# yuriyvnv/speech_transcript_embeddings

Hardware: AMD Instinct MI355X
Metric: audio–text pairs/sec (whole node), 10s@16kHz + 64-tok, 1/2/4/8 MI355X (higher is better)
Workload: dtype bf16; 1 GPU; c2: global batch 64 = 1 GPU x 1 micro-batch(es) of 64 pairs, each pair 10s@16kHz audio + 64-tok clean + 64-tok corrupt; w2v-bert-2.0 Conformer 24L + XLM-R-base 12L, 3+3 unfrozen; GPU fbank -> fwd -> InfoNCE -> bwd -> allreduce -> clip+AdamW; global_batch=64, local_batch=64, micro_batch=64, accumulation_steps=1, seq_len_audio_frames=499, seq_len_text=64, parallelism=dp1

## Files before the change

### speech_transcript_embeddings_amd/csrc/layernorm.hip

```cpp
#include "common.h"
#include "../../include/ste.h"

namespace {

constexpr int NT = 256;

template <int MAXC>
STE_DEV void load_row(const void* base, bool is_bf16, int64_t ld, int row, int cols, int lane, float (&v)[MAXC * 4]) {
#pragma unroll
  for (int c = 0; c < MAXC; ++c) {
    int col = (lane + c * 64) * 4;
    f32x4 x = {0.f, 0.f, 0.f, 0.f};
    if (col < cols) {
      if (is_bf16) x = load_bf16x4((const bf16*)base + (int64_t)row * ld + col);
      else x = *reinterpret_cast<const f32x4*>((const float*)base + (int64_t)row * ld + col);
    }
#pragma unroll
    for (int e = 0; e < 4; ++e) v[c * 4 + e] = x[e];
  }
}

template <int MAXC>
struct LnParams {
  f32x4 g[MAXC], b[MAXC];
  STE_DEV void load(const float* gamma, const float* beta, int cols, int lane) {
#pragma unroll
    for (int c = 0; c < MAXC; ++c) {
      const int col = (lane + c * 64) * 4;
      g[c] = col < cols ? *reinterpret_cast<const f32x4*>(gamma + col) : f32x4{0.f, 0.f, 0.f, 0.f};
      b[c] = (beta && col < cols) ? *reinterpret_cast<const f32x4*>(beta + col) : f32x4{0.f, 0.f, 0.f, 0.f};
    }
  }
};

template <int MAXC>
STE_DEV void ln_fwd_row(const ste_ln_fwd_args& a, const LnParams<MAXC>& pr, int row, int lane, float (&v)[MAXC * 4]) {
  const float inv_n = 1.0f / (float)a.cols;
  const uint32_t thresh = (uint32_t)(a.drop_p * 4294967296.0);
  const float inv_keep = a.drop_p > 0.f ? 1.0f / (1.0f - a.drop_p) : 1.0f;
  float s = 0.f;
#pragma unroll
  for (int i = 0; i < MAXC * 4; ++i) s += v[i];
  const float mean = wave_sum(s) * inv_n;
  float q = 0.f;
#pragma unroll
  for (int c = 0; c < MAXC; ++c) {
    int col = (lane + c * 64) * 4;
    if (col < a.cols) {
#pragma unroll
      for (int e = 0; e < 4; ++e) { float d = v[c * 4 + e] - mean; q += d * d; }
    }
  }
  const float rstd = rsqrtf(wave_sum(q) * inv_n + a.eps);
  if (lane == 0) { a.mean[row] = mean; a.rstd[row] = rstd; }
  const float rs = a.row_scale ? a.row_scale[row] : 1.0f;
#pragma unroll
  for (int c = 0; c < MAXC; ++c) {
    int col = (lane + c * 64) * 4;
    if (col >= a.cols) continue;
    const f32x4 g = pr.g[c], b = pr.b[c];
    f32x4 y;
#pragma unroll
    for (int e = 0; e < 4; ++e) {
      float t = ((v[c * 4 + e] - mean) * rstd * g[e] + b[e]) * rs;
      if (a.act == STE_ACT_SWISH) t = swish_f(t);
      if (a.drop_p > 0.f) t *= drop_scale(a.seed, (uint64_t)row * a.cols + col + e, thresh, inv_keep);
      y[e] = t;
      v[c * 4 + e] = t;
    }
    if (a.y) *reinterpret_cast<f32x4*>(a.y + (int64_t)row * a.ldy + col) = y;
    if (a.ylo) store_bf16x4_split((bf16*)a.yb + (int64_t)row * a.ldyb + col, (bf16*)a.ylo + (int64_t)row * a.ldylo + col, y);
    else if (a.yb) store_bf16x4((bf16*)a.yb + (int64_t)row * a.ldyb + col, y);
    if (a.q8) {
      float am = fmaxf(fmaxf(fabsf(y[0]), fabsf(y[1])), fmaxf(fabsf(y[2]), fabsf(y[3])));
      am = fmaxf(am, dpp_f<0xB1>(am));
      am = fmaxf(am, dpp_f<0x4E>(am));
      am = fmaxf(am, dpp_f<0x141>(am));
      const int ex = mx8_exp(am);
      const float inv = ldexpf(1.0f, -ex);
      uint32_t w = 0;
      w = __builtin_amdgcn_cvt_pk_fp8_f32(fminf(fmaxf(y[0] * inv, -448.f), 448.f),
                                          fminf(fmaxf(y[1] * inv, -448.f), 448.f), w, false);
      w = __builtin_amdgcn_cvt_pk_fp8_f32(fminf(fmaxf(y[2] * inv, -448.f), 448.f),
                                          fminf(fmaxf(y[3] * inv, -448.f), 448.f), w, true);
      *reinterpret_cast<uint32_t*>((uint8_t*)a.q8 + (int64_t)row * a.ldq8 + col) = w;
      if ((lane & 7) == 0) ((uint8_t*)a.q8s)[(int64_t)row * (a.cols >> 5) + (col >> 5)] = (uint8_t)(ex + 127);
    }
  }
}

template <int MAXC>
__global__ __launch_bounds__(NT) void ln_fwd_kernel(ste_ln_fwd_args a) {
  const int lane = threadIdx.x & 63;
  const int wave = blockIdx.x * (NT / 64) + (threadIdx.x >> 6);
  const int nwaves = gridDim.x * (NT / 64);
  LnParams<MAXC> pa;
  pa.load(a.gamma, a.beta, a.cols, lane);
  for (int row = wave; row < a.rows; row += nwaves) {
    float v[MAXC * 4];
    load_row<MAXC>(a.x, a.x_bf16, a.ldx, row, a.cols, lane, v);
    ln_fwd_row<MAXC>(a, pa, row, lane, v);
  }
}

template <int MAXC, bool LEAN = false>
__global__ __launch_bounds__(NT) void ln_fwd_pair_kernel(ste_ln_fwd_args a, ste_ln_fwd_args b) {
  const int lane = threadIdx.x & 63;
  const int wave = blockIdx.x * (NT / 64) + (threadIdx.x >> 6);
  const int nwaves = gridDim.x * (NT / 64);
  if constexpr (LEAN) {
    for (int row = wave; row < a.rows; row += nwaves) {
      float v[MAXC * 4];
      load_row<MAXC>(a.x, a.x_bf16, a.ldx, row, a.cols, lane, v);
      const float *ga = a.gamma, *ba = a.beta, *gb = b.gamma, *bb = b.beta;
      asm volatile("" : "+s"(ga), "+s"(ba), "+s"(gb), "+s"(bb));
      {
        LnParams<MAXC> pa;
        pa.load(ga, ba, a.cols, lane);
        ln_fwd_row<MAXC>(a, pa, row, lane, v);
      }
      LnParams<MAXC> pb;
      pb.load(gb, bb, b.cols, lane);
      ln_fwd_row<MAXC>(b, pb, row, lane, v);
    }
  } else {
    LnParams<MAXC> pa;
    pa.load(a.gamma, a.beta, a.cols, lane);
    LnParams<MAXC> pb;
    pb.load(b.gamma, b.beta, b.cols, lane);
    float v[MAXC * 4], nx[MAXC * 4];
    if (wave < a.rows) load_row<MAXC>(a.x, a.x_bf16, a.ldx, wave, a.cols, lane, v);
    for (int row = wave; row < a.rows; row += nwaves) {
      if (row + nwaves < a.rows) load_row<MAXC>(a.x, a.x_bf16, a.ldx, row + nwaves, a.cols, lane, nx);
      ln_fwd_row<MAXC>(a, pa, row, lane, v);
      ln_fwd_row<MAXC>(b, pb, row, lane, v);
#pragma unroll
      for (int i = 0; i < MAXC * 4; ++i) v[i] = nx[i];
    }
  }
}
bool ln_fwd_pair_lean() {
  static int v = -1;
  if (v < 0) {
    const char* e = STE_AB_ENV("STE_LN_FWD_PAIR");
    v = (e && e[0] == 'p') ? 0 : 1;
  }
  return v == 1;
}

template <int MAXC>
struct LnAcc {
  float dg[MAXC * 4], db[MAXC * 4], dsm[MAXC * 4];
  STE_DEV void zero() {
#pragma unroll
    for (int i = 0; i < MAXC * 4; ++i) { dg[i] = 0.f; db[i] = 0.f; dsm[i] = 0.f; }
  }
};

template <int MAXC, bool PRE, bool DRPRE = PRE>
STE_DEV void ln_bwd_row(const ste_ln_bwd_args& a, int row, int lane, float (&x)[MAXC * 4], float (&g)[MAXC * 4],
                        const float* dr, const LnParams<MAXC>* pr, LnAcc<MAXC>& acc) {
  const float inv_n = 1.0f / (float)a.cols;
  const uint32_t thresh = (uint32_t)(a.drop_p * 4294967296.0);
  const float inv_keep = a.drop_p > 0.f ? 1.0f / (1.0f - a.drop_p) : 1.0f;
  const uint32_t in_thresh = (uint32_t)(a.in_drop_p * 4294967296.0);
  const float in_inv_keep = a.in_drop_p > 0.f ? 1.0f / (1.0f - a.in_drop_p) : 1.0f;
  const float mean = a.mean[row], rstd = a.rstd[row];
  const float rs = a.row_scale ? a.row_scale[row] : 1.0f;
  float s1 = 0.f, s2 = 0.f;
#pragma unroll
  for (int c = 0; c < MAXC; ++c) {
    int col = (lane + c * 64) * 4;
    if (col >= a.cols) continue;
    f32x4 gm, bt = {0.f, 0.f, 0.f, 0.f};
    if constexpr (PRE) {
      gm = pr->g[c];
      bt = pr->b[c];
    } else {
      gm = *reinterpret_cast<const f32x4*>(a.gamma + col);
      if (a.act == STE_ACT_SWISH) bt = *reinterpret_cast<const f32x4*>(a.beta + col);
    }
#pragma unroll
    for (int e = 0; e < 4; ++e) {
      const int i = c * 4 + e;
      const float xh = (x[i] - mean) * rstd;
      float gi = g[i];
      if (a.in_drop_p > 0.f) gi *= drop_scale(a.in_seed, (uint64_t)row * a.cols + col + e, in_thresh, in_inv_keep);
      if (a.act == STE_ACT_SWISH) gi *= swish_d((xh * gm[e] + bt[e]) * rs);
      gi *= rs;
      acc.dg[i] += gi * xh;
      acc.db[i] += gi;
      const float gg = gi * gm[e];
      g[i] = gg;
      x[i] = xh;
      s1 += gg;
      s2 += gg * xh;
    }
  }
  s1 = wave_sum(s1) * inv_n;
  s2 = wave_sum(s2) * inv_n;
  const float ors = a.out_row_scale ? a.out_row_scale[row] : 1.0f;
#pragma unroll
  for (int c = 0; c < MAXC; ++c) {
    int col = (lane + c * 64) * 4;
    if (col >= a.cols) continue;
    f32x4 d;
#pragma unroll
    for (int e = 0; e < 4; ++e) {
      const int i = c * 4 + e;
      d[e] = rstd * (g[i] - s1 - x[i] * s2);
    }
    if (a.dres) {
      if (DRPRE) {
#pragma unroll
        for (int e = 0; e < 4; ++e) d[e] += dr[c * 4 + e];
      } else {
        d += *reinterpret_cast<const f32x4*>(a.dres + (int64_t)row * a.lddres + col);
      }
    }
    if (a.dx) *reinterpret_cast<f32x4*>(a.dx + (int64_t)row * a.lddx + col) = d;
    if (a.dxb || a.dsum) {
      f32x4 o = d * (a.out_scale * ors);
      if (a.drop_p > 0.f) {
#pragma unroll
        for (int e = 0; e < 4; ++e) o[e] *= drop_scale(a.seed, (uint64_t)row * a.cols + col + e, thresh, inv_keep);
      }
      if (a.dxb) store_bf16x4((bf16*)a.dxb + (int64_t)row * a.lddxb + col, o);
#pragma unroll
      for (int e = 0; e < 4; ++e) acc.dsm[c * 4 + e] += o[e];
    }
#pragma unroll
    for (int e = 0; e < 4; ++e) g[c * 4 + e] = d[e];
  }
}

template <int MAXC>
STE_DEV void ln_flush(const ste_ln_bwd_args& a, const LnAcc<MAXC>& acc, float (*red)[MAXC * 4 * 64], int lane,
                      int wid) {
  float* const outs[3] = {a.dgamma, a.dbeta, a.dsum};
#pragma unroll
  for (int k = 0; k < 3; ++k) {
    if (!outs[k]) continue;
    const float* src = k == 0 ? acc.dg : (k == 1 ? acc.db : acc.dsm);
    __syncthreads();
#pragma unroll
    for (int i = 0; i < MAXC * 4; ++i) red[wid][(i >> 2) * 256 + lane * 4 + (i & 3)] = src[i];
    __syncthreads();
    float* part = a.ws ? a.ws + ((int64_t)k * gridDim.x + blockIdx.x) * a.cols : nullptr;
    for (int j = threadIdx.x; j < MAXC * 256; j += NT) {
      const int c = j >> 8, rem = j & 255;
      const int col = (c * 64 + (rem >> 2)) * 4 + (rem & 3);
      if (col >= a.cols) continue;
      float sum = 0.f;
#pragma unroll
      for (int w = 0; w < NT / 64; ++w) sum += red[w][j];
      if (part) part[col] = sum;
      else atomicAdd(outs[k] + col, sum);
    }
  }
}

constexpr int CS_CW = 16, CS_SL = 1024 / CS_CW;
__global__ __launch_bounds__(1024) void ln_colsum_kernel(const float* __restrict__ ws, int nblk, int cols,
                                                         float* dgamma, float* dbeta, float* dsum) {
  float* const out = blockIdx.y == 0 ? dgamma : (blockIdx.y == 1 ? dbeta : dsum);
  if (!out) return;
  __shared__ float red[CS_SL][CS_CW];
  const int c = threadIdx.x % CS_CW, sl = threadIdx.x / CS_CW;
  const int col = blockIdx.x * CS_CW + c;
  float acc = 0.f;
  if (col < cols) {
    const float* p = ws + (int64_t)blockIdx.y * nblk * cols + col;
    int b = sl;
    for (; b + 7 * CS_SL < nblk; b += 8 * CS_SL) {
      float v[8];
#pragma unroll
      for (int u = 0; u < 8; ++u) v[u] = p[(int64_t)(b + CS_SL * u) * cols];
#pragma unroll
      for (int u = 0; u < 8; ++u) acc += v[u];
    }
    for (; b < nblk; b += CS_SL) acc += p[(int64_t)b * cols];
  }
  red[sl][c] = acc;
  __syncthreads();
  if (sl == 0 && col < cols) {
    float t = red[0][c];
    for (int k = 1; k < CS_SL; ++k) t += red[k][c];
    out[col] += t;
  }
}

template <int MAXC, bool REDUCE>
__global__ __launch_bounds__(NT, REDUCE ? 3 : 1) void ln_bwd_kernel(ste_ln_bwd_args a) {
  __shared__ float red[REDUCE ? NT / 64 : 1][REDUCE ? MAXC * 4 * 64 : 1];
  const int lane = threadIdx.x & 63, wid = threadIdx.x >> 6;
  const int wave = blockIdx.x * (NT / 64) + wid;
  const int nwaves = gridDim.x * (NT / 64);
  LnAcc<MAXC> acc;
  acc.zero();
  LnParams<MAXC> pa;
  if constexpr (!REDUCE) pa.load(a.gamma, a.act == STE_ACT_SWISH ? a.beta : nullptr, a.cols, lane);
  for (int row = wave; row < a.rows; row += nwaves) {
    float x[MAXC * 4], g[MAXC * 4], dr[MAXC * 4];
    load_row<MAXC>(a.x, a.x_bf16, a.ldx, row, a.cols, lane, x);
    load_row<MAXC>(a.dy, a.dy_bf16, a.lddy, row, a.cols, lane, g);
    if (a.dres) load_row<MAXC>(a.dres, false, a.lddres, row, a.cols, lane, dr);
    if constexpr (REDUCE) ln_bwd_row<MAXC, false, true>(a, row, lane, x, g, dr, nullptr, acc);
    else ln_bwd_row<MAXC, true>(a, row, lane, x, g, dr, &pa, acc);
  }
  if constexpr (REDUCE) ln_flush<MAXC>(a, acc, red, lane, wid);
}

template <int MAXC, bool REDUCE>
__global__ __launch_bounds__(NT, REDUCE ? 1 : 4) void ln_bwd_pair_kernel(ste_ln_bwd_args a, ste_ln_bwd_args b) {
  __shared__ float red[REDUCE ? NT / 64 : 1][REDUCE ? MAXC * 4 * 64 : 1];
  const int lane = threadIdx.x & 63, wid = threadIdx.x >> 6;
  const int wave = blockIdx.x * (NT / 64) + wid;
  const int nwaves = gridDim.x * (NT / 64);
  LnAcc<MAXC> acc_a, acc_b;
  acc_a.zero();
  acc_b.zero();
  for (int row = wave; row < a.rows; row += nwaves) {
    float x[MAXC * 4], g[MAXC * 4], dr[MAXC * 4];
    load_row<MAXC>(b.x, b.x_bf16, b.ldx, row, b.cols, lane, x);
    load_row<MAXC>(b.dy, b.dy_bf16, b.lddy, row, b.cols, lane, g);
    if (!REDUCE && b.dres) load_row<MAXC>(b.dres, false, b.lddres, row, b.cols, lane, dr);
    ln_bwd_row<MAXC, false, !REDUCE>(b, row, lane, x, g, dr, nullptr, acc_b);
    load_row<MAXC>(a.x, a.x_bf16, a.ldx, row, a.cols, lane, x);
    ln_bwd_row<MAXC, false>(a, row, lane, x, g, nullptr, nullptr, acc_a);
  }
  if constexpr (REDUCE) {
    ln_flush<MAXC>(b, acc_b, red, lane, wid);
    ln_flush<MAXC>(a, acc_a, red, lane, wid);
  }
}

inline int grid_for(int rows, int cap = 1024) {
  int g = (rows + 3) / 4;
  return g < cap ? g : cap;
}
constexpr int LN_REDUCE_BLOCKS = 768, LN_PAIR_REDUCE_BLOCKS = 512;
inline int grid_bwd(const ste_ln_bwd_args& a, bool reduce) {
  return grid_for(a.rows, reduce ? LN_REDUCE_BLOCKS : 1024);
}
inline bool ws_ok(const ste_ln_bwd_args& a, int nblk) {
  return !a.ws || a.ws_floats >= 3 * (int64_t)nblk * a.cols;
}
inline void colsum(const ste_ln_bwd_args& a, int nblk, hipStream_t s) {
  if (!a.ws || !(a.dgamma || a.dbeta || a.dsum)) return;
  hipLaunchKernelGGL(ln_colsum_kernel, dim3((unsigned)((a.cols + CS_CW - 1) / CS_CW), 3), dim3(1024), 0, s, (const float*)a.ws,
                     nblk, a.cols, a.dgamma, a.dbeta, a.dsum);
}

}

extern "C" int ste_layernorm_fwd(const ste_ln_fwd_args* a, void* stream) {
  if (!a || a->rows <= 0 || a->cols <= 0 || (a->cols & 3) || a->cols > 2048 || !a->mean || !a->rstd)
    return STE_ERR_ARG;
  if (a->ylo && !a->yb) return STE_ERR_ARG;
  if (a->q8 && (!a->q8s || (a->cols & 127) || a->ldq8 < a->cols || (a->ldq8 & 3) || (((uintptr_t)a->q8) & 3)))
    return STE_ERR_SHAPE;
  hipStream_t s = (hipStream_t)stream;
  dim3 grid(grid_for(a->rows));
  if (a->cols <= 256) hipLaunchKernelGGL(ln_fwd_kernel<1>, grid, dim3(NT), 0, s, *a);
  else if (a->cols <= 1024) hipLaunchKernelGGL(ln_fwd_kernel<4>, grid, dim3(NT), 0, s, *a);
  else hipLaunchKernelGGL(ln_fwd_kernel<8>, grid, dim3(NT), 0, s, *a);
  STE_CHECK_LAUNCH();
  return 0;
}

extern "C" int ste_layernorm_fwd_pair(const ste_ln_fwd_args* a, const ste_ln_fwd_args* b, void* stream) {
  if (!a || !b || a->rows <= 0 || a->cols <= 0 || (a->cols & 3) || a->cols > 1024 || b->rows != a->rows ||
      b->cols != a->cols || !a->mean || !a->rstd || !b->mean || !b->rstd)
    return STE_ERR_ARG;
  for (const ste_ln_fwd_args* t : {a, b}) {
    if (t->ylo && !t->yb) return STE_ERR_ARG;
    if (t->q8 && (!t->q8s || (t->cols & 127) || t->ldq8 < t->cols || (t->ldq8 & 3) || (((uintptr_t)t->q8) & 3)))
      return STE_ERR_SHAPE;
  }
  hipStream_t s = (hipStream_t)stream;
  dim3 grid(grid_for(a->rows));
  if (a->cols <= 256) hipLaunchKernelGGL(ln_fwd_pair_kernel<1>, grid, dim3(NT), 0, s, *a, *b);
  else if (ln_fwd_pair_lean()) hipLaunchKernelGGL((ln_fwd_pair_kernel<4, true>), grid, dim3(NT), 0, s, *a, *b);
  else hipLaunchKernelGGL(ln_fwd_pair_kernel<4>, grid, dim3(NT), 0, s, *a, *b);
  STE_CHECK_LAUNCH();
  return 0;
}

extern "C" int ste_layernorm_bwd_pair(const ste_ln_bwd_args* a, const ste_ln_bwd_args* b, void* stream) {
  if (!a || !b || a->rows <= 0 || a->cols <= 0 || (a->cols & 3) || a->cols > 1024 || b->rows != a->rows ||
      b->cols != a->cols)
    return STE_ERR_ARG;
  if ((a->act == STE_ACT_SWISH && !a->beta) || (b->act == STE_ACT_SWISH && !b->beta)) return STE_ERR_ARG;
  hipStream_t s = (hipStream_t)stream;
  const bool reduce = a->dgamma || a->dbeta || a->dsum || b->dgamma || b->dbeta || b->dsum;
  const bool use_ws = (a->ws || !(a->dgamma || a->dbeta || a->dsum)) && (b->ws || !(b->dgamma || b->dbeta || b->dsum));
  const int nblk = grid_for(a->rows, reduce ? LN_PAIR_REDUCE_BLOCKS : 1024);
  if (reduce && use_ws && (!ws_ok(*a, nblk) || !ws_ok(*b, nblk))) return STE_ERR_ARG;
  ste_ln_bwd_args aa = *a, bb = *b;
  if (!use_ws) aa.ws = bb.ws = nullptr;
  const dim3 grid(nblk);
  if (a->cols <= 256) {
    if (reduce) hipLaunchKernelGGL((ln_bwd_pair_kernel<1, true>), grid, dim3(NT), 0, s, aa, bb);
    else hipLaunchKernelGGL((ln_bwd_pair_kernel<1, false>), grid, dim3(NT), 0, s, aa, bb);
  } else {
    if (reduce) hipLaunchKernelGGL((ln_bwd_pair_kernel<4, true>), grid, dim3(NT), 0, s, aa, bb);
    else hipLaunchKernelGGL((ln_bwd_pair_kernel<4, false>), grid, dim3(NT), 0, s, aa, bb);
  }
  STE_CHECK_LAUNCH();
  if (reduce && use_ws) {
    colsum(bb, nblk, s);
    colsum(aa, nblk, s);
    STE_CHECK_LAUNCH();
  }
  return 0;
}

extern "C" int ste_layernorm_bwd(const ste_ln_bwd_args* a, void* stream) {
  if (!a || a->rows <= 0 || a->cols <= 0 || (a->cols & 3) || a->cols > 1024) return STE_ERR_ARG;
  if (a->act == STE_ACT_SWISH && !a->beta) return STE_ERR_ARG;
  hipStream_t s = (hipStream_t)stream;
  const bool reduce = a->dgamma || a->dbeta || a->dsum;
  const int nblk = grid_bwd(*a, reduce);
  if (reduce && !ws_ok(*a, nblk)) return STE_ERR_ARG;
  const dim3 grid(nblk);
  if (a->cols <= 256) {
    if (reduce) hipLaunchKernelGGL((ln_bwd_kernel<1, true>), grid, dim3(NT), 0, s, *a);
    else hipLaunchKernelGGL((ln_bwd_kernel<1, false>), grid, dim3(NT), 0, s, *a);
  } else {
    if (reduce) hipLaunchKernelGGL((ln_bwd_kernel<4, true>), grid, dim3(NT), 0, s, *a);
    else hipLaunchKernelGGL((ln_bwd_kernel<4, false>), grid, dim3(NT), 0, s, *a);
  }
  STE_CHECK_LAUNCH();
  if (reduce) {
    colsum(*a, nblk, s);
    STE_CHECK_LAUNCH();
  }
  return 0;
}

extern "C" int64_t ste_layernorm_bwd_ws_floats(int rows, int cols) {
  return rows <= 0 || cols <= 0 ? 0 : 3 * (int64_t)grid_for(rows, LN_REDUCE_BLOCKS) * cols;
}
```

Before: 494.7 pairs/s.

## Add LDS ring-buffered LayerNorm forward pair kernel using global_load_lds prefetch

Adds a new paired LayerNorm forward kernel that prefetches the next row of fp32 input (plus row scales) straight into a per-wave LDS slot with global_load_lds. It keeps gamma/beta for both norms in shared memory instead of registers, and uses explicit vmcnt waits so the next row's loads overlap the current row's compute and stores. The aim is to hide load latency and lower register pressure (launch bounds allow 4 blocks). It is used by default for fp32 inputs with 512–1024 columns and no fp8 output, and the old path stays selectable through an env var. It relies on hand-written asm waitcnt counting, which is fragile if the store count estimate is wrong.

```diff
diff --git a/profiles/ln_dma_probe.py b/profiles/ln_dma_probe.py
--- /dev/null
+++ b/profiles/ln_dma_probe.py
@@ -0,0 +1,88 @@
+import argparse
+import json
+import os
+import statistics
+import sys
+from pathlib import Path
+
+import torch
+
+sys.path.insert(0, str(Path(__file__).resolve().parents[1]))
+from speech_transcript_embeddings_amd import _lib, ops
+
+M, D = 31936, 1024
+BF16 = torch.bfloat16
+
+
+def timed(fn, iters):
+    fn()
+    torch.cuda.synchronize()
+    e0, e1 = torch.cuda.Event(enable_timing=True), torch.cuda.Event(enable_timing=True)
+    e0.record()
+    for _ in range(iters):
+        fn()
+    e1.record()
+    torch.cuda.synchronize()
+    return round(e0.elapsed_time(e1) * 1e3 / iters, 2)
+
+
+def cases():
+    dev = "cuda"
+    torch.manual_seed(0)
+    x = torch.randn(M, D, device=dev)
+    x5s = torch.randn(M, 2 * D, device=dev)
+    g, b = 1 + 0.1 * torch.randn(D, device=dev), 0.1 * torch.randn(D, device=dev)
+    g2, b2 = 1 + 0.1 * torch.randn(D, device=dev), 0.1 * torch.randn(D, device=dev)
+    rs = (torch.rand(M, device=dev) > 0.1).float()
+    y = torch.empty(M, D, device=dev)
+    yb2 = torch.empty(M, D, device=dev, dtype=BF16)
+    ys = torch.empty(M, 2 * D, device=dev, dtype=BF16)
+    mean, rstd = torch.empty(M, device=dev), torch.empty(M, device=dev)
+    m2, r2 = torch.empty(M, device=dev), torch.empty(M, device=dev)
+    c = {}
+    c["fwd_pair ring: y+yb+ylo | yb"] = (1, lambda: ops.layernorm_fwd_pair(
+        dict(x=x, gamma=g, beta=b, eps=1e-5, y=y, yb=ys[:, :D], ylo=ys[:, D:], mean=mean, rstd=rstd),
+        dict(gamma=g2, beta=b2, eps=1e-5, yb=yb2, mean=m2, rstd=r2)), (y, ys, yb2, mean, rstd, m2, r2))
+    c["fwd_pair ring: wide x, y+yb+ylo | yb row_scale"] = (1, lambda: ops.layernorm_fwd_pair(
+        dict(x=x5s[:, :D], gamma=g, beta=b, eps=1e-5, y=y, yb=ys[:, :D], ylo=ys[:, D:], mean=mean, rstd=rstd),
+        dict(gamma=g2, beta=b2, eps=1e-5, yb=yb2, mean=m2, rstd=r2, row_scale=rs)), (y, ys, yb2, mean, rstd, m2, r2))
+    return c
+
+
+def main():
+    ap = argparse.ArgumentParser()
+    ap.add_argument("--iters", type=int, default=20)
+    ap.add_argument("--alt", type=int, default=7)
+    ap.add_argument("--out", default=None)
+    a = ap.parse_args()
+    assert _lib.AB_BUILD, "run with STE_LIB=.../libste_ab.so (python -m speech_transcript_embeddings_amd._build --ab)"
+    lines = []
+    for name, (bit, fn, outs) in cases().items():
+        old, new = [], []
+        for _ in range(a.alt):
+            os.environ["STE_LN_DMA"] = "0"
+            old.append(timed(fn, a.iters))
+            os.environ["STE_LN_DMA"] = str(bit)
+            new.append(timed(fn, a.iters))
+        os.environ["STE_LN_DMA"] = "0"
+        fn()
+        ref = [t.clone() for t in outs]
+        for t in outs:
+            t.fill_(3.0)
+        os.environ["STE_LN_DMA"] = str(bit)
+        fn()
+        torch.cuda.synchronize()
+        same = all(torch.equal(r, t) for r, t in zip(ref, outs))
+        res = dict(case=name, rows=M, cols=D, parent_us=old, ring_us=new, parent_median=statistics.median(old),
+                   ring_median=statistics.median(new), parent_spread=round(max(old) - min(old), 2),
+                   ring_spread=round(max(new) - min(new), 2), bit_identical=same)
+        res["speedup"] = round(res["parent_median"] / res["ring_median"], 3)
+        lines.append(json.dumps(res))
+        print(lines[-1], flush=True)
+    if a.out:
+        Path(a.out).parent.mkdir(parents=True, exist_ok=True)
+        Path(a.out).write_text("\n".join(lines) + "\n")
+
+
+if __name__ == "__main__":
+    main()
diff --git a/speech_transcript_embeddings_amd/csrc/layernorm.hip b/speech_transcript_embeddings_amd/csrc/layernorm.hip
--- a/speech_transcript_embeddings_amd/csrc/layernorm.hip
+++ b/speech_transcript_embeddings_amd/csrc/layernorm.hip
@@ -1,9 +1,15 @@
+#include <cstdlib>
 #include "common.h"
 #include "../../include/ste.h"
 
 namespace {
 
 constexpr int NT = 256;
+
+inline int grid_for(int rows, int cap = 1024) {
+  int g = (rows + 3) / 4;
+  return g < cap ? g : cap;
+}
 
 template <int MAXC>
 STE_DEV void load_row(const void* base, bool is_bf16, int64_t ld, int row, int cols, int lane, float (&v)[MAXC * 4]) {
@@ -31,10 +37,13 @@
       b[c] = (beta && col < cols) ? *reinterpret_cast<const f32x4*>(beta + col) : f32x4{0.f, 0.f, 0.f, 0.f};
     }
   }
+  STE_DEV void get(int c, f32x4& gc, f32x4& bc) const { gc = g[c]; bc = b[c]; }
 };
 
-template <int MAXC>
-STE_DEV void ln_fwd_row(const ste_ln_fwd_args& a, const LnParams<MAXC>& pr, int row, int lane, float (&v)[MAXC * 4]) {
+STE_DEV float fwd_rs(const ste_ln_fwd_args& a, int row) { return a.row_scale ? a.row_scale[row] : 1.0f; }
+template <int MAXC, class Params>
+STE_DEV void ln_fwd_row(const ste_ln_fwd_args& a, const Params& pr, int row, int lane, float (&v)[MAXC * 4],
+                        float rs) {
   const float inv_n = 1.0f / (float)a.cols;
   const uint32_t thresh = (uint32_t)(a.drop_p * 4294967296.0);
   const float inv_keep = a.drop_p > 0.f ? 1.0f / (1.0f - a.drop_p) : 1.0f;
@@ -53,12 +62,12 @@
   }
   const float rstd = rsqrtf(wave_sum(q) * inv_n + a.eps);
   if (lane == 0) { a.mean[row] = mean; a.rstd[row] = rstd; }
-  const float rs = a.row_scale ? a.row_scale[row] : 1.0f;
 #pragma unroll
   for (int c = 0; c < MAXC; ++c) {
     int col = (lane + c * 64) * 4;
     if (col >= a.cols) continue;
-    const f32x4 g = pr.g[c], b = pr.b[c];
+    f32x4 g, b;
+    pr.get(c, g, b);
     f32x4 y;
 #pragma unroll
     for (int e = 0; e < 4; ++e) {
@@ -99,7 +108,7 @@
   for (int row = wave; row < a.rows; row += nwaves) {
     float v[MAXC * 4];
     load_row<MAXC>(a.x, a.x_bf16, a.ldx, row, a.cols, lane, v);
-    ln_fwd_row<MAXC>(a, pa, row, lane, v);
+    ln_fwd_row<MAXC>(a, pa, row, lane, v, fwd_rs(a, row));
   }
 }
 
@@ -117,11 +126,11 @@
       {
         LnParams<MAXC> pa;
         pa.load(ga, ba, a.cols, lane);
-        ln_fwd_row<MAXC>(a, pa, row, lane, v);
+        ln_fwd_row<MAXC>(a, pa, row, lane, v, fwd_rs(a, row));
       }
       LnParams<MAXC> pb;
       pb.load(gb, bb, b.cols, lane);
-      ln_fwd_row<MAXC>(b, pb, row, lane, v);
+      ln_fwd_row<MAXC>(b, pb, row, lane, v, fwd_rs(b, row));
     }
   } else {
     LnParams<MAXC> pa;
@@ -132,8 +141,8 @@
     if (wave < a.rows) load_row<MAXC>(a.x, a.x_bf16, a.ldx, wave, a.cols, lane, v);
     for (int row = wave; row < a.rows; row += nwaves) {
       if (row + nwaves < a.rows) load_row<MAXC>(a.x, a.x_bf16, a.ldx, row + nwaves, a.cols, lane, nx);
-      ln_fwd_row<MAXC>(a, pa, row, lane, v);
-      ln_fwd_row<MAXC>(b, pb, row, lane, v);
+      ln_fwd_row<MAXC>(a, pa, row, lane, v, fwd_rs(a, row));
+      ln_fwd_row<MAXC>(b, pb, row, lane, v, fwd_rs(b, row));
 #pragma unroll
       for (int i = 0; i < MAXC * 4; ++i) v[i] = nx[i];
     }
@@ -148,6 +157,118 @@
   return v == 1;
 }
 
+typedef __attribute__((address_space(3))) const char lds_cchar;
+STE_DEV uint32_t lds_off(const void* p) { return (uint32_t)(uintptr_t)(lds_cchar*)p; }
+
+template <int N>
+STE_DEV void lds_read_chunks(uint32_t off, f32x4 (&r)[N]) {
+  static_assert(N >= 2 && N <= 4, "2..4 chunks");
+  if constexpr (N == 2)
+    asm volatile("ds_read_b128 %0, %2\n\tds_read_b128 %1, %2 offset:1024\n\ts_waitcnt lgkmcnt(0)"
+                 : "=&v"(r[0]), "=&v"(r[1]) : "v"(off) : "memory");
+  else if constexpr (N == 3)
+    asm volatile("ds_read_b128 %0, %3\n\tds_read_b128 %1, %3 offset:1024\n\tds_read_b128 %2, %3 offset:2048\n\t"
+                 "s_waitcnt lgkmcnt(0)"
+                 : "=&v"(r[0]), "=&v"(r[1]), "=&v"(r[2]) : "v"(off) : "memory");
+  else
+    asm volatile("ds_read_b128 %0, %4\n\tds_read_b128 %1, %4 offset:1024\n\tds_read_b128 %2, %4 offset:2048\n\t"
+                 "ds_read_b128 %3, %4 offset:3072\n\ts_waitcnt lgkmcnt(0)"
+                 : "=&v"(r[0]), "=&v"(r[1]), "=&v"(r[2]), "=&v"(r[3]) : "v"(off) : "memory");
+}
+template <int NCH>
+struct LnParamsLds {
+  uint32_t off;
+  STE_DEV void get(int c, f32x4& gc, f32x4& bc) const {
+    asm volatile("ds_read_b128 %0, %2\n\tds_read_b128 %1, %3\n\ts_waitcnt lgkmcnt(0)"
+                 : "=&v"(gc), "=&v"(bc) : "v"(off + c * 1024), "v"(off + (NCH + c) * 1024) : "memory");
+  }
+};
+STE_DEV float lds_read_f32(uint32_t off) {
+  float r;
+  asm volatile("ds_read_b32 %0, %1\n\ts_waitcnt lgkmcnt(0)" : "=&v"(r) : "v"(off) : "memory");
+  return r;
+}
+STE_DEV void wait_vmcnt(int n) {
+#define STE_VMC(k) case k: asm volatile("s_waitcnt vmcnt(" #k ")" ::: "memory"); break;
+  switch (n) {
+    STE_VMC(1) STE_VMC(2) STE_VMC(3) STE_VMC(4) STE_VMC(5) STE_VMC(6) STE_VMC(7) STE_VMC(8) STE_VMC(9) STE_VMC(10)
+    STE_VMC(11) STE_VMC(12) STE_VMC(13) STE_VMC(14) STE_VMC(15) STE_VMC(16) STE_VMC(17) STE_VMC(18) STE_VMC(19)
+    STE_VMC(20) STE_VMC(21) STE_VMC(22) STE_VMC(23) STE_VMC(24) STE_VMC(25) STE_VMC(26) STE_VMC(27) STE_VMC(28)
+    default: asm volatile("s_waitcnt vmcnt(0)" ::: "memory"); break;
+  }
+#undef STE_VMC
+}
+
+template <int NCH>
+__global__ __launch_bounds__(NT, 4) void ln_fwd_pair_ring_kernel(ste_ln_fwd_args a, ste_ln_fwd_args b, int nstores) {
+  __shared__ __attribute__((aligned(16))) char ring[NT / 64][NCH * 1024];
+  __shared__ __attribute__((aligned(16))) float rsc[NT / 64][2][64];
+  __shared__ __attribute__((aligned(16))) float par[4][NCH * 256];
+  const int lane = threadIdx.x & 63, wid = threadIdx.x >> 6;
+  const int wave = blockIdx.x * (NT / 64) + wid;
+  const int nwaves = gridDim.x * (NT / 64);
+  const float* const psrc[4] = {a.gamma, a.beta, b.gamma, b.beta};
+#pragma unroll
+  for (int k = 0; k < 4; ++k)
+    for (int i = threadIdx.x * 4; i < NCH * 256; i += NT * 4)
+      *reinterpret_cast<f32x4*>(&par[k][i]) =
+          psrc[k] ? *reinterpret_cast<const f32x4*>(psrc[k] + i) : f32x4{0.f, 0.f, 0.f, 0.f};
+  __syncthreads();
+  char* const slot = ring[wid];
+  const uint32_t soff = lds_off(slot) + lane * 16, rsoff = lds_off(rsc[wid]) + lane * 4;
+  const uint32_t poff = lds_off(par) + lane * 16;
+  auto issue = [&](int row) {
+    const float* src = (const float*)a.x + (int64_t)row * a.ldx + lane * 4;
+#pragma unroll
+    for (int c = 0; c < NCH; ++c)
+      __builtin_amdgcn_global_load_lds((const void*)(src + c * 256), (lds_void*)(slot + c * 1024), 16, 0, 0);
+    if (a.row_scale) __builtin_amdgcn_global_load_lds((const void*)(a.row_scale + row), (lds_void*)rsc[wid][0], 4, 0, 0);
+    if (b.row_scale) __builtin_amdgcn_global_load_lds((const void*)(b.row_scale + row), (lds_void*)rsc[wid][1], 4, 0, 0);
+  };
+  int row = wave;
+  if (row >= a.rows) return;
+  issue(row);
+  asm volatile("s_waitcnt vmcnt(0)" ::: "memory");
+  for (;;) {
+    f32x4 t[NCH];
+    lds_read_chunks<NCH>(soff, t);
+    const float rsa = a.row_scale ? lds_read_f32(rsoff) : 1.0f;
+    const float rsb = b.row_scale ? lds_read_f32(rsoff + 256) : 1.0f;
+    const int nxt = row + nwaves;
+    if (nxt < a.rows) issue(nxt);
+    float v[NCH * 4];
+#pragma unroll
+    for (int c = 0; c < NCH; ++c)
+#pragma unroll
+      for (int e = 0; e < 4; ++e) v[c * 4 + e] = t[c][e];
+    ln_fwd_row<NCH>(a, LnParamsLds<NCH>{poff}, row, lane, v, rsa);
+    ln_fwd_row<NCH>(b, LnParamsLds<NCH>{poff + 2 * NCH * 1024}, row, lane, v, rsb);
+    if (nxt >= a.rows) break;
+    row = nxt;
+    wait_vmcnt(nstores);
+  }
+}
+inline int ring_stores(const ste_ln_fwd_args& a) {
+  return 2 + (a.cols / 256) * ((a.y ? 1 : 0) + (a.ylo ? 2 : (a.yb ? 1 : 0)));
+}
+inline bool ring_ok(const ste_ln_fwd_args& a, bool needs_x) {
+  if (a.cols < 512 || a.cols > 1024 || (a.cols & 255) || a.q8) return false;
+  return !needs_x || (!a.x_bf16 && !(a.ldx & 3) && !(((uintptr_t)a.x) & 15));
+}
+inline bool ln_pair_ring() {
+  const char* e = STE_AB_ENV("STE_LN_DMA");
+  return !e || atoi(e) != 0;
+}
+inline void launch_fwd_pair_ring(const ste_ln_fwd_args& a, const ste_ln_fwd_args& b, hipStream_t s) {
+  const dim3 grid(grid_for(a.rows));
+  const int n = ring_stores(a) + ring_stores(b);
+  switch (a.cols / 256) {
+    case 2: hipLaunchKernelGGL(ln_fwd_pair_ring_kernel<2>, grid, dim3(NT), 0, s, a, b, n); break;
+    case 3: hipLaunchKernelGGL(ln_fwd_pair_ring_kernel<3>, grid, dim3(NT), 0, s, a, b, n); break;
+    default: hipLaunchKernelGGL(ln_fwd_pair_ring_kernel<4>, grid, dim3(NT), 0, s, a, b, n); break;
+  }
+}
+
 template <int MAXC>
 struct LnAcc {
   float dg[MAXC * 4], db[MAXC * 4], dsm[MAXC * 4];
@@ -157,16 +278,19 @@
   }
 };
 
+struct LnRowStat { float mean, rstd, rs, ors; };
+STE_DEV LnRowStat bwd_stat(const ste_ln_bwd_args& a, int row) {
+  return {a.mean[row], a.rstd[row], a.row_scale ? a.row_scale[row] : 1.0f, a.out_row_scale ? a.out_row_scale[row] : 1.0f};
+}
 template <int MAXC, bool PRE, bool DRPRE = PRE>
 STE_DEV void ln_bwd_row(const ste_ln_bwd_args& a, int row, int lane, float (&x)[MAXC * 4], float (&g)[MAXC * 4],
-                        const float* dr, const LnParams<MAXC>* pr, LnAcc<MAXC>& acc) {
+                        const float* dr, const LnParams<MAXC>* pr, LnAcc<MAXC>& acc, const LnRowStat& st) {
   const float inv_n = 1.0f / (float)a.cols;
   const uint32_t thresh = (uint32_t)(a.drop_p * 4294967296.0);
   const float inv_keep = a.drop_p > 0.f ? 1.0f / (1.0f - a.drop_p) : 1.0f;
   const uint32_t in_thresh = (uint32_t)(a.in_drop_p * 4294967296.0);
   const float in_inv_keep = a.in_drop_p > 0.f ? 1.0f / (1.0f - a.in_drop_p) : 1.0f;
-  const float mean = a.mean[row], rstd = a.rstd[row];
-  const float rs = a.row_scale ? a.row_scale[row] : 1.0f;
+  const float mean = st.mean, rstd = st.rstd, rs = st.rs;
   float s1 = 0.f, s2 = 0.f;
 #pragma unroll
   for (int c = 0; c < MAXC; ++c) {
@@ -199,7 +323,7 @@
   }
   s1 = wave_sum(s1) * inv_n;
   s2 = wave_sum(s2) * inv_n;
-  const float ors = a.out_row_scale ? a.out_row_scale[row] : 1.0f;
+  const float ors = st.ors;
 #pragma unroll
   for (int c = 0; c < MAXC; ++c) {
     int col = (lane + c * 64) * 4;
@@ -305,8 +429,8 @@
     load_row<MAXC>(a.x, a.x_bf16, a.ldx, row, a.cols, lane, x);
     load_row<MAXC>(a.dy, a.dy_bf16, a.lddy, row, a.cols, lane, g);
     if (a.dres) load_row<MAXC>(a.dres, false, a.lddres, row, a.cols, lane, dr);
-    if constexpr (REDUCE) ln_bwd_row<MAXC, false, true>(a, row, lane, x, g, dr, nullptr, acc);
-    else ln_bwd_row<MAXC, true>(a, row, lane, x, g, dr, &pa, acc);
+    if constexpr (REDUCE) ln_bwd_row<MAXC, false, true>(a, row, lane, x, g, dr, nullptr, acc, bwd_stat(a, row));
+    else ln_bwd_row<MAXC, true>(a, row, lane, x, g, dr, &pa, acc, bwd_stat(a, row));
   }
   if constexpr (REDUCE) ln_flush<MAXC>(a, acc, red, lane, wid);
 }
@@ -325,9 +449,9 @@
     load_row<MAXC>(b.x, b.x_bf16, b.ldx, row, b.cols, lane, x);
     load_row<MAXC>(b.dy, b.dy_bf16, b.lddy, row, b.cols, lane, g);
     if (!REDUCE && b.dres) load_row<MAXC>(b.dres, false, b.lddres, row, b.cols, lane, dr);
-    ln_bwd_row<MAXC, false, !REDUCE>(b, row, lane, x, g, dr, nullptr, acc_b);
+    ln_bwd_row<MAXC, false, !REDUCE>(b, row, lane, x, g, dr, nullptr, acc_b, bwd_stat(b, row));
     load_row<MAXC>(a.x, a.x_bf16, a.ldx, row, a.cols, lane, x);
-    ln_bwd_row<MAXC, false>(a, row, lane, x, g, nullptr, nullptr, acc_a);
+    ln_bwd_row<MAXC, false>(a, row, lane, x, g, nullptr, nullptr, acc_a, bwd_stat(a, row));
   }
   if constexpr (REDUCE) {
     ln_flush<MAXC>(b, acc_b, red, lane, wid);
@@ -335,10 +459,6 @@
   }
 }
 
-inline int grid_for(int rows, int cap = 1024) {
-  int g = (rows + 3) / 4;
-  return g < cap ? g : cap;
-}
 constexpr int LN_REDUCE_BLOCKS = 768, LN_PAIR_REDUCE_BLOCKS = 512;
 inline int grid_bwd(const ste_ln_bwd_args& a, bool reduce) {
   return grid_for(a.rows, reduce ? LN_REDUCE_BLOCKS : 1024);
@@ -381,6 +501,8 @@
   hipStream_t s = (hipStream_t)stream;
   dim3 grid(grid_for(a->rows));
   if (a->cols <= 256) hipLaunchKernelGGL(ln_fwd_pair_kernel<1>, grid, dim3(NT), 0, s, *a, *b);
+  else if (ln_pair_ring() && ln_fwd_pair_lean() && ring_ok(*a, true) && ring_ok(*b, false))
+    launch_fwd_pair_ring(*a, *b, s);
   else if (ln_fwd_pair_lean()) hipLaunchKernelGGL((ln_fwd_pair_kernel<4, true>), grid, dim3(NT), 0, s, *a, *b);
   else hipLaunchKernelGGL(ln_fwd_pair_kernel<4>, grid, dim3(NT), 0, s, *a, *b);
   STE_CHECK_LAUNCH();
```

Measured after the change: 497.2 pairs/s (median of 6 runs). No clear change (+0.5%).
